# mit-gfx/recfilter

Hardware: AMD Instinct MI355X
Metric: Mpixels/s + achieved HBM GB/s, 16384^2 order-2 x/y Gaussian IIR (higher is better)
Workload: dtype f32; 1 GPU; cfg3: 16384x16384 f32 x1 plane(s) per GPU, 4 scans, clamped border; exchange=none, interior_beside_collective=False, steps_in_flight=1, backend=none, rccl_ranks=0

## Files before the change

include/recfilter_amd.h:

```cpp
#ifndef RECFILTER_AMD_H
#define RECFILTER_AMD_H

#include <stddef.h>
#include <stdint.h>

#ifdef __cplusplus
extern "C" {
#endif

#define RF_MAX_DIMS    3
#define RF_MAX_ORDER   32
#define RF_MAX_SCANS   32
#define RF_MAX_PLANES  16
#define RF_DEVICE_HOST_ONLY (-2)

typedef enum {
    RF_OK = 0,
    RF_ERR_INVALID_ARG = 1,
    RF_ERR_UNSUPPORTED = 2,
    RF_ERR_HIP = 3,
    RF_ERR_NOMEM = 4,
    RF_ERR_STATE = 5
} rf_status;

// ... 31 lines not shown
#define RF_PLAN_FORCE_EXCHANGE  0x01u
#define RF_PLAN_TILED_ONLY      0x02u
#define RF_PLAN_NO_CASCADE      0x04u
#define RF_PLAN_NO_SECTIONS     0x08u
#define RF_PLAN_NO_PLANE_BATCH  0x10u
#define RF_PLAN_STREAM_PASS1    0x20u
#define RF_PLAN_STAGED_PASS1    0x40u
#define RF_PLAN_LATE_EXCHANGE   0x80u
#define RF_PLAN_SERIAL_UNTILED  0x01000000u
#define RF_PLAN_MFMA_PASS1      0x02000000u
#define RF_PLAN_WALK_PASS1      0x04000000u
#define RF_PLAN_NO_OVERLAP      0x08000000u
#define RF_PLAN_INPLACE_Z       0x10000000u
#define RF_PLAN_FULL_CARRY_SCAN 0x20000000u
#define RF_PLAN_STAGE_HALF      0x40000000u
#define RF_PLAN_ALL_FLAGS       0x7f0000ffu
#define RF_PLAN_TILE_ROWS(n)    (((uint32_t)(n) & 0xffu) << 8)
#define RF_PLAN_TILE_PLANES(n)  (((uint32_t)(n) & 0xffu) << 16)

#define RF_ABI 3u

typedef struct {
    int32_t  ndim;
    uint32_t abi;
    int64_t  extent[RF_MAX_DIMS];
    int32_t  dtype;
    int32_t  n_planes;
    int32_t  border;
    int32_t  n_scans;
    const rf_scan_desc *scans;
    int32_t  tile[RF_MAX_DIMS];
// ... 71 lines not shown
```

recfilter_amd/capi.py:

```python
from __future__ import annotations

import ctypes
import os
import subprocess

_PKG = os.path.dirname(os.path.abspath(__file__))
LIB_PATH = os.environ.get("RECFILTER_AMD_LIB") or os.path.join(_PKG, "librecfilter_amd.so")
CSRC = os.path.join(_PKG, "csrc")

RF_MAX_DIMS = 3
RF_MAX_ORDER = 32
RF_ABI = 3
RF_MAX_SCANS = 32
RF_MAX_PLANES = 16
RF_DEVICE_HOST_ONLY = -2

RF_OK, RF_ERR_INVALID_ARG, RF_ERR_UNSUPPORTED, RF_ERR_HIP, RF_ERR_NOMEM, RF_ERR_STATE = range(6)
RF_F32, RF_F64, RF_I32, RF_I16, RF_F16, RF_BF16 = range(6)
RF_BORDER_ZERO, RF_BORDER_CLAMP = 0, 1
RF_POINTWISE_PRE, RF_POINTWISE_POST = 1, 2
RF_IN_PIXEL, RF_IN_U8, RF_IO_U8 = 0, 1, 2
RF_BUFFER_TABLE, RF_BUFFER_ZEROED, RF_BUFFER_SCRATCH = range(3)
BUFFER_KIND_NAMES = {RF_BUFFER_TABLE: "table", RF_BUFFER_ZEROED: "zeroed", RF_BUFFER_SCRATCH: "scratch"}
RF_PATH_AUTO, RF_PATH_UNTILED, RF_PATH_TILED_GENERIC, RF_PATH_TILED_FUSED, RF_PATH_TILED_OVERLAPPED, RF_PATH_TILED_MATRIX = range(6)
RF_PLAN_FORCE_EXCHANGE, RF_PLAN_TILED_ONLY, RF_PLAN_NO_CASCADE, RF_PLAN_NO_SECTIONS = 0x01, 0x02, 0x04, 0x08
RF_PLAN_NO_PLANE_BATCH, RF_PLAN_STREAM_PASS1, RF_PLAN_STAGED_PASS1, RF_PLAN_LATE_EXCHANGE = 0x10, 0x20, 0x40, 0x80
RF_PLAN_SERIAL_UNTILED = 0x01000000
RF_PLAN_MFMA_PASS1 = 0x02000000
RF_PLAN_WALK_PASS1 = 0x04000000
RF_PLAN_NO_OVERLAP = 0x08000000
RF_PLAN_INPLACE_Z = 0x10000000
RF_PLAN_FULL_CARRY_SCAN = 0x20000000
RF_PLAN_STAGE_HALF = 0x40000000


def RF_PLAN_TILE_ROWS(n: int) -> int:
    return (int(n) & 0xff) << 8


def RF_PLAN_TILE_PLANES(n: int) -> int:
    return (int(n) & 0xff) << 16


PATH_NAMES = {RF_PATH_AUTO: "auto", RF_PATH_UNTILED: "untiled",
              RF_PATH_TILED_GENERIC: "tiled_generic", RF_PATH_TILED_FUSED: "tiled_fused",
              RF_PATH_TILED_OVERLAPPED: "tiled_overlapped", RF_PATH_TILED_MATRIX: "tiled_matrix"}

EXPORTED_SYMBOLS = [
# ... 110 lines not shown
```

recfilter_amd/csrc/kernels_fused.h:

```cpp
#pragma once

#include <hip/hip_runtime.h>

#include <cstdint>

#include "kernels.h"
#include "pixel.h"
#include "rf_internal.h"

namespace rf {

constexpr int kFusedTX = 256;
constexpr int kFusedSeg = 16;
constexpr int kFusedThreads = 256;
constexpr int kFusedMaxK = 3;
constexpr int kFusedMaxMod = 8;
constexpr int kFusedMaxScans = 4;

template <typename Acc>
struct FusedScan {
    int32_t causal;
    Acc b;
    Acc a[kFusedMaxK];
    Acc R[kFusedMaxK][kFusedSeg];
// ... 36 lines not shown
    const Acc *y_nb_W;
    const Acc *x_incoming;
    int32_t pw_flags;
    Acc pre_s, pre_b, post_f, post_i, post_b;
    int32_t plane_batch;
    int32_t tx0, ty0, gx, gy;
    int32_t xcd_contig;
    int32_t mod_form;
    const void *in_planes[kFusedMaxPlanes];
    void *out_planes[kFusedMaxPlanes];
    int32_t yt_tile_major;
    int32_t yt_parts;
    int64_t yt_part_stride;
    const Acc *ytp;
    int64_t lin_limit;
    __host__ __device__ int64_t yt_index(int j, int ty, int r, int K, int64_t line) const {
        if (yt_tile_major)
            return ((((int64_t)ty * (NXP * NZ / kFusedTX) + (line >> 8)) * ny + j) * K + r) * kFusedTX + (line & 255);
        return (((int64_t)j * MY + ty) * K + r) * (NXP * NZ) + line;
    }
};

template <typename Acc>
struct StridedArgs {
    int64_t n, inner, lines;
    int32_t M;
    int32_t n_scans;
    int32_t clamped, first_is_border, last_is_border;
    int32_t mod_form;
    FusedScanY<Acc> scans[kFusedMaxScans];
// ... 47 lines not shown
int launch_fused_pass2_tall(int K, const void *src, int src_kind, P *dst, const FusedArgs<typename PixelTraits<P>::Acc> &a,
                            hipStream_t stream);
int launch_fused_pass2_u8(int K, int TY, const uint8_t *src, uint8_t *dst, const FusedArgs<float> &a, hipStream_t stream);
int launch_fused_pass2_tall_u8(int K, const uint8_t *src, uint8_t *dst, const FusedArgs<float> &a, hipStream_t stream);
template <typename P>
int launch_fused_tails(int K, int TY, const void *src, bool src_u8, const FusedArgs<typename PixelTraits<P>::Acc> &a,
                       const typename PixelTraits<P>::Acc *Hx, const typename PixelTraits<P>::Acc *Hy,
                       hipStream_t stream);
bool stream_tails_applicable(int K, int TY, bool src_u8, int pw_flags, int last_cols, int last_rows, int64_t n_tiles, int MX,
                             int64_t NZ, int nxk, int nyk, int mode );
int launch_stream_tails(int K, const float *src, const FusedArgs<float> &a, const float *Hx, const float *Hy, hipStream_t stream);
bool mfma_tails_applicable(int K, int TY, bool src_u8, int pw_flags, int last_cols, int last_rows, int64_t lin_limit, int nx, int ny,
                           int mode, bool narrow = false );
template <typename PI>
int launch_mfma_tails(int K, int TY, const PI *src, const FusedArgs<float> &a, const float *Hx, const float *Hy, hipStream_t stream);
struct WalkArgs {
    float *ytp;
    int64_t part_stride;
    float *zt;
    const float *HzT;
    int32_t TY, TZ, MZ;
    int32_t parts_log2;
    int32_t z_first_border, z_last_border;
    int32_t nzk, KZ;
    int32_t tall;
    float *xt2;
};
bool walk_tails_applicable(int K, int TY, int nx, int ny, int nz, int KZ, int TZ, int last_cols, int last_rows);
int launch_walk_tails(int K, const float *src, const FusedArgs<float> &a, const WalkArgs &wa, const float *Hx, const float *Hy,
                      hipStream_t stream);
// ... 6 lines not shown
```

recfilter_amd/csrc/kernels_fused_tall.hip:

```cpp
#include <atomic>
#include <type_traits>

#include "kernels.h"
#include "kernels_fused.h"
#include "scan_device.h"

namespace rf {

namespace {

constexpr int kTallTY = 128;
constexpr int kHalfRows = 64;

template <typename P, int K, bool EDGE, typename PI, int YPAT, bool EARLY, bool XFIX>
__global__ void __launch_bounds__(kFusedThreads, 2)
fused_pass2_tall_kernel(const PI *__restrict__ src, P *__restrict__ dst, FusedArgs<typename PixelTraits<P>::Acc> a) {
    using Acc = typename PixelTraits<P>::Acc;
    using A4 = typename Vec4<Acc>::type;
    extern __shared__ __attribute__((aligned(16))) unsigned char lds_raw[];
    Acc *tile = reinterpret_cast<Acc *>(lds_raw);
    A4 *tile4 = reinterpret_cast<A4 *>(lds_raw);
    constexpr int TY = kTallTY, TL = kHalfRows, NR = TL / 16;

    const int t = threadIdx.x;
    int bx = (int)blockIdx.x, by = (int)blockIdx.y;
    if (a.xcd_contig) {
        const unsigned gxn = gridDim.x, total = gxn * gridDim.y;
        unsigned b = (unsigned)by * gxn + (unsigned)bx;
        b = (b & 7u) * (total >> 3) + (b >> 3);
// ... 43 lines not shown
#pragma unroll
        for (int r = 0; r < K; r++) CY[j][r] = Acc(0);
        if (j < a.ny) {
            const bool causal = a.ys[j].causal != 0;
            const bool tile_first = causal ? (ty == 0) : (ty == a.MY - 1);
            if (tile_first) {
#pragma unroll
                for (int r = 0; r < K; r++) CY[j][r] = a.y_incoming[((int64_t)j * K + r) * Ly + line];
            } else {
                const int tp = causal ? ty - 1 : ty + 1;
#pragma unroll
                for (int r = 0; r < K; r++) CY[j][r] = a.yt[a.yt_index(j, tp, r, K, line)];
            }
        }
    }
    Acc yin[kFusedMaxScans][K];
    if (a.y_apply != nullptr) {
#pragma unroll
        for (int q = 0; q < kFusedMaxScans; q++)
#pragma unroll
            for (int o = 0; o < K; o++) yin[q][o] = q < a.ny ? a.y_incoming[((int64_t)q * K + o) * Ly + line] : Acc(0);
    } else if (a.y_nb_W != nullptr && ty < a.MY - 1) {
#pragma unroll
        for (int o = 0; o < K; o++) yin[0][o] = a.yt[a.yt_index(0, ty, o, K, line)];
    }
    auto apply_entering_carries = [&]() {
        if (a.y_nb_W != nullptr) {
            if (ty < a.MY - 1) {
                const int v = (ty + 1 == a.MY - 1) ? 2 : 0;
                const Acc *Wm = a.y_nb_W + ((v * a.ny + 0) * a.ny + 1) * K * K;
#pragma unroll
                for (int r = 0; r < K; r++)
#pragma unroll
                    for (int o = 0; o < K; o++) CY[1][r] = CY[1][r] + Wm[r * K + o] * yin[0][o];
            }
            return;
        }
        if (a.y_apply == nullptr) return;
#pragma unroll
        for (int j = 0; j < kFusedMaxScans; j++) {
            if (j < a.ny) {
// ... 7 lines not shown
#pragma unroll
                        for (int q = 0; q <= j; q++) {
                            const Acc *Ym = a.y_apply + ((((int64_t)q * a.ny + j) * a.MY + tp) * K + r) * K;
#pragma unroll
                            for (int o = 0; o < K; o++) add = add + Ym[o] * yin[q][o];
                        }
                        CY[j][r] = CY[j][r] + add;
                    }
                }
            }
        }
    };

    Acc *cx_lds = tile + TL * kFusedTX;
    Acc CX[2][kFusedMaxScans][NR][K];
#pragma unroll
    for (int h = 0; h < 2; h++) {
        const int64_t line0 = (int64_t)ty * TY + TL * h + slot + a.NYP * z;
#pragma unroll
        for (int s = 0; s < kFusedMaxScans; s++) {
#pragma unroll
            for (int n = 0; n < NR; n++)
#pragma unroll
                for (int j = 0; j < K; j++) CX[h][s][n][j] = Acc(0);
            if (s < a.nx) {
                const bool causal = a.xs[s].causal != 0;
                const bool tile_first = causal ? (tx == 0) : (tx == a.MX - 1);
                const bool first_lane = causal ? (l == 0) : (l == last_lane);
                if (first_lane) {
                    const int tp = causal ? tx - 1 : tx + 1;
                    const Acc *cp = tile_first ? a.x_incoming + (int64_t)s * K * Lx : a.xt + ((int64_t)s * a.MX + tp) * K * Lx;
#pragma unroll
                    for (int n = 0; n < NR; n++)
#pragma unroll
                        for (int j = 0; j < K; j++) CX[h][s][n][j] = cp[j * Lx + line0 + 16 * n];
                }
            }
        }
    }
    auto park_carries = [&]() {
#pragma unroll
        for (int h = 0; h < 2; h++)
#pragma unroll
            for (int s = 0; s < kFusedMaxScans; s++) {
                if (s < a.nx) {
                    const bool causal = a.xs[s].causal != 0;
                    const bool first_lane = causal ? (l == 0) : (l == last_lane);
                    if (first_lane) {
#pragma unroll
                        for (int n = 0; n < NR; n++)
#pragma unroll
                            for (int j = 0; j < K; j++) cx_lds[(((h * kFusedMaxScans + s) * NR + n) * K + j) * 16 + slot] = CX[h][s][n][j];
                    }
                }
            }
// ... 179 lines not shown
            } else
            if constexpr (packed_stores<P>::value) {
#pragma unroll
                for (int i = 0; i < TY; i += 2)
                    store_row_pair<P>(dpb, (uint32_t)t, (uint32_t)i, row_bytes, col[i], col[i + 1], (uint32_t)(EDGE ? rows_here : TY));
            } else
#pragma unroll
            for (int i = 0; i < TY; i++)
                if (!EDGE || i < rows_here)
                    __builtin_nontemporal_store(PixelTraits<P>::store(col[i]),
                                                reinterpret_cast<P *>(dpb + ((uint32_t)t * (uint32_t)sizeof(P) + (uint32_t)i * row_bytes)));
        }
    }
}

template <typename P, int K, bool EDGE, typename PI, int YPAT, bool EARLY, bool XFIX = false>
int launch_tall_pat(const PI *src, P *dst, const FusedArgs<typename PixelTraits<P>::Acc> &a, hipStream_t stream) {
    using Acc = typename PixelTraits<P>::Acc;
    const size_t lds = ((size_t)kHalfRows * kFusedTX + 2 * kFusedMaxScans * (kHalfRows / 16) * K * 16 + (size_t)a.ny * K * kFusedTX) * sizeof(Acc);
    const size_t lds_max = ((size_t)kHalfRows * kFusedTX + 2 * kFusedMaxScans * (kHalfRows / 16) * K * 16 + (size_t)kFusedMaxScans * K * kFusedTX) * sizeof(Acc);
    static std::atomic<bool> attr_set[64];
    int dev = 0;
    RF_HIP_CHECK(hipGetDevice(&dev));
    std::atomic<bool> &done = attr_set[dev & 63];
    if (!done.load(std::memory_order_acquire)) {
        RF_HIP_CHECK(hipFuncSetAttribute(reinterpret_cast<const void *>(&fused_pass2_tall_kernel<P, K, EDGE, PI, YPAT, EARLY, XFIX>),
                                         hipFuncAttributeMaxDynamicSharedMemorySize, (int)lds_max));
        done.store(true, std::memory_order_release);
    }
    dim3 grid((unsigned)(a.gx > 0 ? a.gx : a.MX), (unsigned)(a.gy > 0 ? a.gy : a.MY), (unsigned)a.NZ);
    FusedArgs<Acc> aa = a;
    aa.xcd_contig = (a.row_bytes % 128u != 0 && (grid.x * grid.y) % 8u == 0 && grid.x * grid.y >= 2048u) ? 1 : 0;
    hipLaunchKernelGGL((fused_pass2_tall_kernel<P, K, EDGE, PI, YPAT, EARLY, XFIX>), grid, dim3(kFusedThreads), lds, stream, src, dst, aa);
    RF_HIP_CHECK(hipGetLastError());
    return RF_OK;
}

template <typename P, int K, bool EDGE, typename PI>
int launch_tall_impl(const PI *src, P *dst, const FusedArgs<typename PixelTraits<P>::Acc> &a, hipStream_t stream) {
    const int pat = a.mod_form ? 0 : (a.ny == 1 && a.ys[0].causal != 0) ? 1 : (a.ny == 2 && a.ys[0].causal != 0 && a.ys[1].causal == 0) ? 2 : 0;
    bool early = !EDGE && pat > 0;
    if constexpr (!PixelTraits<P>::is_integer) early = early && (a.pw_flags & 2) == 0;
    const int xpat = a.mod_form ? 0 : (a.nx == 1 && a.xs[0].causal != 0) ? 1 : (a.nx == 2 && a.xs[0].causal != 0 && a.xs[1].causal == 0) ? 2 : 0;
    if constexpr (!EDGE) {
        if (early && pat == 1 && xpat == 1) return launch_tall_pat<P, K, EDGE, PI, 1, true, true>(src, dst, a, stream);
        if (early && pat == 2 && xpat == 2) return launch_tall_pat<P, K, EDGE, PI, 2, true, true>(src, dst, a, stream);
        if (early && pat == 1) return launch_tall_pat<P, K, EDGE, PI, 1, true>(src, dst, a, stream);
        if (early && pat == 2) return launch_tall_pat<P, K, EDGE, PI, 2, true>(src, dst, a, stream);
    }
    if (pat == 1) return launch_tall_pat<P, K, EDGE, PI, 1, false>(src, dst, a, stream);
    if (pat == 2) return launch_tall_pat<P, K, EDGE, PI, 2, false>(src, dst, a, stream);
    return launch_tall_pat<P, K, EDGE, PI, 0, false>(src, dst, a, stream);
}

template <int K, bool EDGE, typename PI>
int launch_tall_widen(const PI *src, float *dst, const FusedArgs<float> &a, hipStream_t stream) {
    if (a.mod_form || (a.pw_flags & 2) || a.plane_batch || a.y_nb_W != nullptr || a.y_apply != nullptr) {
        set_error("fused pass 2: a 16-bit source with an f32 destination is the x/y stage of an unsharded volume (no epilogue, no sections)");
// ... 100 lines not shown
```

recfilter_amd/csrc/kernels_tails.hip:

```cpp
#include <cstdlib>
#include <type_traits>

#include "kernels.h"
#include "kernels_fused.h"
#include "scan_device.h"

namespace rf {

namespace {


typedef float F2 __attribute__((ext_vector_type(2)));
typedef float F4 __attribute__((ext_vector_type(4)));

template <typename P, int K, int TY, typename PI, int MODE = 0, bool YM = false>
__global__ void __launch_bounds__(kFusedThreads)
fused_tails_kernel(const PI *__restrict__ src, FusedArgs<typename PixelTraits<P>::Acc> a,
                   const typename PixelTraits<P>::Acc *__restrict__ Hx,
                   const typename PixelTraits<P>::Acc *__restrict__ Hy) {
    using Acc = typename PixelTraits<P>::Acc;
    using A4 = typename Vec4<Acc>::type;
    constexpr int kTailRows = sizeof(Acc) == 8 ? 16 : 32;
    __shared__ __attribute__((aligned(16))) Acc tile[kTailRows * kFusedTX];
    extern __shared__ __attribute__((aligned(16))) unsigned char hx_raw[];
// ... 582 lines not shown
                const int64_t y = ybase + 4 * c4;
                A4 v = *reinterpret_cast<const A4 *>(a.xt + (((int64_t)s * a.MX + tx_i) * K + r) * Lx + y);
                if (s == 1 && tx_i > 0) {
                    const int vt = (tx_i == a.MX - 1) ? 2 : 0;
                    const Acc *Wm = Wx + ((vt * a.nx + 0) * a.nx + 1) * K * K + r * K;
#pragma unroll
                    for (int m = 0; m < K; m++) {
                        const A4 p = *reinterpret_cast<const A4 *>(a.xt + ((int64_t)(tx_i - 1) * K + m) * Lx + y);
                        const Acc w = Wm[m];
                        v.x = v.x + w * p.x; v.y = v.y + w * p.y; v.z = v.z + w * p.z; v.w = v.w + w * p.w;
                    }
                }
                *reinterpret_cast<A4 *>(xt_done + (((int64_t)s * a.MX + tx_i) * K + r) * Lx + y) = v;
            }
        }
    }
}

}

template <typename P>
int launch_fused_tails(int K, int TY, const void *src, bool src_u8, const FusedArgs<typename PixelTraits<P>::Acc> &a,
                       const typename PixelTraits<P>::Acc *Hx, const typename PixelTraits<P>::Acc *Hy,
                       hipStream_t stream) {
    if (a.MX <= 0 || a.MY <= 0 || a.NZ <= 0) return RF_OK;
    if (a.NZ > 65535 || a.MY > 65535) { set_error("fused path: grid too large"); return RF_ERR_UNSUPPORTED; }
    dim3 grid((unsigned)a.MX, (unsigned)a.MY, (unsigned)a.NZ);
    static const size_t pad_bytes = RF_KNOB("RF_TAILS_PAD_LDS") ? (size_t)atoi(RF_KNOB("RF_TAILS_PAD_LDS")) : 0;
    const size_t hx_bytes = (size_t)(a.nx > 0 ? a.nx : 1) * K * kFusedTX * sizeof(typename PixelTraits<P>::Acc) + pad_bytes;
    const size_t hy_bytes = (size_t)((a.ny * K + 3) & ~3) * 9 * 16;
// ... 125 lines not shown
            if (edge) RF_XSCAN_LAUNCH((Acc, KK, true, true), (Acc, KK, true, true, 0, true), dim3(grid), dim3(256), g_bytes, stream, a, gj, TY, Hy, G);  \
            else      RF_XSCAN_LAUNCH((Acc, KK, false, true), (Acc, KK, false, true, 0, true), dim3(grid), dim3(256), g_bytes, stream, a, gj, TY, Hy, G); \
        } else {                                                                                                           \
            if (edge) RF_XSCAN_LAUNCH((Acc, KK, true, false), (Acc, KK, true, false, 0, true), dim3(grid), dim3(256), g_bytes, stream, a, gj, TY, Hy, G);  \
            else      RF_XSCAN_LAUNCH((Acc, KK, false, false), (Acc, KK, false, false, 0, true), dim3(grid), dim3(256), g_bytes, stream, a, gj, TY, Hy, G); \
        }                                                                                                                  \
        RF_HIP_CHECK(hipGetLastError());                                                                                   \
        return RF_OK;                                                                                                      \
    }
    RF_CASE(1) RF_CASE(2) RF_CASE(3)
#undef RF_CASE
    set_error("xscan rows: unsupported order %d", K);
    return RF_ERR_UNSUPPORTED;
}

template int launch_fused_tails<float>(int, int, const void *, bool, const FusedArgs<float> &, const float *, const float *, hipStream_t);
template int launch_fused_tails<_Float16>(int, int, const void *, bool, const FusedArgs<float> &, const float *, const float *, hipStream_t);
template int launch_fused_tails<__bf16>(int, int, const void *, bool, const FusedArgs<float> &, const float *, const float *, hipStream_t);
template int launch_fused_tails<int32_t>(int, int, const void *, bool, const FusedArgs<uint32_t> &, const uint32_t *,
                                         const uint32_t *, hipStream_t);
template int launch_fused_tails<int16_t>(int, int, const void *, bool, const FusedArgs<uint32_t> &, const uint32_t *,
                                         const uint32_t *, hipStream_t);
template int launch_fused_tails<double>(int, int, const void *, bool, const FusedArgs<double> &, const double *, const double *, hipStream_t);
template int launch_xscan_rows<float>(int, int, const FusedArgs<float> &, const float *, const float *, hipStream_t, const float *, const float *, float *, bool);
template int launch_xscan_rows<uint32_t>(int, int, const FusedArgs<uint32_t> &, const uint32_t *, const uint32_t *, hipStream_t, const uint32_t *, const uint32_t *, uint32_t *, bool);
template int launch_xscan_rows<double>(int, int, const FusedArgs<double> &, const double *, const double *, hipStream_t, const double *, const double *, double *, bool);

}
```

recfilter_amd/csrc/kernels_tails_mfma.hip:

```cpp
#include <atomic>
#include <cstdlib>
#include <type_traits>

#include "kernels.h"
#include "kernels_fused.h"
#include "scan_device.h"

namespace rf {

namespace {

typedef float F2 __attribute__((ext_vector_type(2)));
typedef float F4 __attribute__((ext_vector_type(4)));

constexpr int kRows = 32;
constexpr int kHyPitch4 = 9;

__device__ __forceinline__ float sum_lanes_xor_16_32(float v) {
    typedef unsigned U2 __attribute__((ext_vector_type(2)));
    U2 r = __builtin_amdgcn_permlane16_swap(__float_as_uint(v), __float_as_uint(v), false, false);
    v = __uint_as_float(r[0]) + __uint_as_float(r[1]);
    r = __builtin_amdgcn_permlane32_swap(__float_as_uint(v), __float_as_uint(v), false, false);
    return __uint_as_float(r[0]) + __uint_as_float(r[1]);
}

__device__ __forceinline__ int row_swz(int row, int c) { return c ^ (row & 15) ^ ((c >> 4) & 3); }

template <int K, int TY, int NX, int NY, bool YM, typename PI = float>
__global__ void __launch_bounds__(kFusedThreads, 4)
mfma_tails_kernel(const PI *__restrict__ src, FusedArgs<float> a,
                  const float *__restrict__ Hx,
                  const float *__restrict__ Hy) {
    __shared__ __attribute__((aligned(16))) float tile[kRows * kFusedTX];
    extern __shared__ __attribute__((aligned(16))) unsigned char dyn_raw[];
    F4 *tile4 = reinterpret_cast<F4 *>(tile);
    float *stage = reinterpret_cast<float *>(dyn_raw);
    constexpr int NH = TY / kRows;
    constexpr int NL = kRows / 4;
    constexpr int NGX = NX > 0 ? (NX * K + 3) / 4 : 1;
    constexpr int NGY = NY > 0 ? (NY * K + 3) / 4 : 1;
    constexpr int NYK = NY > 0 ? NY * K : 1;

    const int t = threadIdx.x;
// ... 145 lines not shown
                                c0 = F2{h0[i], h0[i + 1]} * c2 + c0;
                                c1 = F2{h1[i], h1[i + 1]} * c2 + c1;
                            }
                            comb[2 * g] = comb[2 * g] + (c0.x + c0.y);
                            if (2 * g + 1 < NYK) comb[2 * g + 1] = comb[2 * g + 1] + (c1.x + c1.y);
                        }
                    }
                }
            }
        }
    }
    if (nxk > 0) {
        __syncthreads();
        flush_xtails(NH - 1);
    }
    if constexpr (YM) {
        if (nyk > 0) {
            const int64_t line = (int64_t)tx * kFusedTX + (t & ~3) + a.NXP * z;
#pragma unroll
            for (int g = 0; g < NGY; g++) {
                const int jr = 4 * g + (t & 3);
                if (jr < nyk) *reinterpret_cast<F4 *>(a.yt + a.yt_index(jr / K, ty, jr % K, K, line)) = yacc[g];
            }
        }
    } else if (nyk > 0) {
        const int64_t line = (int64_t)tx * kFusedTX + t + a.NXP * z;
#pragma unroll
        for (int jr = 0; jr < NYK; jr++)
            if (jr < nyk) a.yt[a.yt_index(jr / K, ty, jr % K, K, line)] = comb[jr];
    }
// ... 34 lines not shown
    if constexpr (std::is_same<PI, float>::value) {
        RF_CASES(1, 32) RF_CASES(1, 64) RF_CASES(1, 128)
        RF_CASES(2, 32) RF_CASES(2, 64) RF_CASES(2, 128)
        RF_CASES(3, 32) RF_CASES(3, 64) RF_CASES(3, 128)
    } else {
        RF_CASES_PAIRS(2, 32) RF_CASES_PAIRS(2, 64) RF_CASES_PAIRS(2, 128)
        RF_CASES_PAIRS(3, 32) RF_CASE(3, 64, 1, 1) RF_CASES_PAIRS(3, 128)
    }
#undef RF_CASES
#undef RF_CASES_PAIRS
#undef RF_CASE
    set_error("mfma tails: unsupported order %d / tile height %d / %d + %d scans", K, TY, a.nx, a.ny);
    return RF_ERR_UNSUPPORTED;
}

template int launch_mfma_tails<float>(int, int, const float *, const FusedArgs<float> &, const float *, const float *, hipStream_t);
template int launch_mfma_tails<_Float16>(int, int, const _Float16 *, const FusedArgs<float> &, const float *, const float *, hipStream_t);
template int launch_mfma_tails<__bf16>(int, int, const __bf16 *, const FusedArgs<float> &, const float *, const float *, hipStream_t);

}
```

recfilter_amd/csrc/plan_fused.cpp:

```cpp
#include <cmath>
#include <cstring>
#include <memory>

#include "kernels_fused.h"
#include "plan.h"
#include "plan_carry.h"
#include "plan_generic.h"
#include "plan_strided.h"

namespace rf {

namespace {

int fused_order(const rf_plan *plan) {
    return std::max(plan->dims[0].k, plan->ndim > 1 ? plan->dims[1].k : 0);
}

int64_t chained_padded_length(int64_t N) {
    if (N % 8192 == 0) return N;
    for (int64_t nx = 16384; nx >= kFusedTX; nx /= 2) {
        const int64_t g = nx * 32, np = (N + g - 1) / g * g;
        if (np - N <= N / 16) return np;
    }
    return (N + 8191) / 8192 * 8192;
// ... 121 lines not shown
    g.NX = NX; g.NY = NY; g.NZ = NZ; g.nx = nx; g.ny = ny;
    g.TY = TY; g.MX = MX; g.MY = MY; g.TVx = TVx; g.TVy = TVy;
    g.NXP = NXP; g.NYP = NYP; g.Lx = Lx; g.Ly = Ly;
    return g;
}

template <typename S, typename Acc>
struct FusedTables {
    CarryStage<S, Acc> x, y;
    std::vector<FusedScan<Acc>> xs, ys;
    const Acc *G = nullptr;
    const Acc *Hx = nullptr, *Hy = nullptr;
    const Acc *AMx = nullptr, *AMSx = nullptr;
    int chain_S = 1;
    bool nb_x = false, nb_y = false;
    bool nb_x_pair() const { return nb_x && x.n == 2; }
    bool nb_y_pair() const { return nb_y && y.n == 2; }
};

template <typename P, typename S>
int fused_tables(rf_plan *plan, const FusedGeometry &g, FusedTables<S, typename PixelTraits<P>::Acc> &t) {
    using Acc = typename PixelTraits<P>::Acc;
    using Options = typename CarryStage<S, Acc>::Options;
    int status = RF_OK;
    const int K = g.K, nx = g.nx, ny = g.ny;
    const DimInfo &dx = plan->dims[0];
    const DimInfo no_y;
    const DimInfo &dy = g.chained ? no_y : plan->dims[1];
    auto up = [&](const auto &vec) {
        using T = typename std::decay<decltype(vec)>::type::value_type;
// ... 49 lines not shown
                        dG[idx] = table_to_double<S>(Pm[(size_t)xi * K + o]);
                    }
            }
        plan->tables["G_x"] = dG;
    }
    if (ny > 0) {
        if (neighbour_plan) nb_bound_y = neighbour_carry_bound<S>(t.y.tab, dy.scan_ids, plan);
        hHy = table_for_kernels<S, Acc>(plan, build_tail_responses<S>(t.y.tab.scans, K, g.TY, plan->clamped, g.TVy), "H_y");
    }
    t.G = up(hG); t.Hx = up(hHx); t.Hy = up(hHy); t.AMx = up(hAMx); t.AMSx = up(hAMSx);

    const bool full_scan = (plan->flags & RF_PLAN_FULL_CARRY_SCAN) != 0;
    t.nb_x = !full_scan && nb_bound_x >= 0.0 && nb_bound_x <= kNeighbourCarryBound && (nx == 1 || ny > 0);
    t.nb_y = !full_scan && nb_bound_y >= 0.0 && nb_bound_y <= kNeighbourCarryBound && (ny == 1 || g.TY == 128);
    plan->tables["neighbour_carries"] = {nb_bound_x, t.nb_x ? 1.0 : 0.0, nb_bound_y, t.nb_y ? 1.0 : 0.0};
    return status;
}

template <typename Acc>
struct FusedBuffers {
    Acc *xt = nullptr, *yt = nullptr;
    Acc *xt_done = nullptr;
    Acc *xin = nullptr, *yin = nullptr;
    Acc *row_exit = nullptr;
    size_t xt_pp = 0, yt_pp = 0, xin_pp = 0, yin_pp = 0;
    bool merged_cx = false;
};

template <typename S, typename Acc>
int fused_buffers(rf_plan *plan, const FusedGeometry &g, FusedTables<S, Acc> &t, FusedBuffers<Acc> &b) {
// ... 83 lines not shown
        if (batch)
            for (int i = 0; i < plan->n_planes; i++) { a.in_planes[i] = plan->in[i]; a.out_planes[i] = plan->xy_result(i); }
        return a;
    }
};

template <typename Acc>
struct Pass1Args {
    int K = 0, TY = 0;
    const Acc *Hx = nullptr, *Hy = nullptr;
    bool padded = false;
    int stream_mode = 0, mfma_mode = 0;
    WalkArgs walk{};
    std::shared_ptr<WalkHook> walk_hook;
    size_t xt_pp = 0;
};

template <typename P>
int launch_pass1(const rf_plan *plan, int pl, const FusedArgs<typename PixelTraits<P>::Acc> &a,
                 const Pass1Args<typename PixelTraits<P>::Acc> &p) {
    const int K = p.K, TY = p.TY;
    const void *in = p.padded ? plan->pad_in[pl] : plan->in[pl];
    if constexpr (std::is_same<P, float>::value) {
        if (p.walk_hook) {
            WalkArgs wa = p.walk;
            wa.zt = p.walk_hook->zt + (size_t)pl * p.walk_hook->zt_stride;
            if (wa.xt2) wa.xt2 += (size_t)pl * p.xt_pp;
            if (wa.ytp) wa.ytp = const_cast<float *>(a.ytp);
            else wa.ytp = a.yt;
            return launch_walk_tails(K, (const float *)plan->in[pl], a, wa, p.Hx, p.Hy, plan->stream);
        }
        if (a.lin_limit == 0 && stream_tails_applicable(K, TY, plan->pw.in_u8, a.pw_flags, a.last_cols, a.last_rows, (int64_t)a.MX * a.MY * a.NZ, a.MX,
                                        a.NZ, a.nx * K, a.ny * K, p.stream_mode))
            return launch_stream_tails(K, (const float *)in, a, p.Hx, p.Hy, plan->stream);
        if (mfma_tails_applicable(K, TY, plan->pw.in_u8, a.pw_flags, a.last_cols, a.last_rows, a.lin_limit, a.nx, a.ny, p.mfma_mode))
            return launch_mfma_tails<float>(K, TY, (const float *)in, a, p.Hx, p.Hy, plan->stream);
    }
    if constexpr (is_half_pixel<P>::value) {
// ... 56 lines not shown
            for (int e = 0; e < kFusedMaxMod; e++) fbase.ys[j].mod_g[e] = t.ys[j].mod_g[e];
        }
        fargs.b = b;
        fargs.batch = g.batch;
        t.y.dev.base.tile_major = fbase.yt_tile_major;
    }

    int add_pass1() {
        int status = RF_OK;
        rf_plan *const plan = this->plan;
        Pass1Args<Acc> p1a;
        p1a.K = g.K; p1a.TY = g.TY; p1a.Hx = t.Hx; p1a.Hy = t.Hy; p1a.padded = g.padded;
        p1a.stream_mode = (plan->flags & RF_PLAN_STREAM_PASS1) ? 1 : (plan->flags & RF_PLAN_STAGED_PASS1) ? -1 : 0;
        p1a.mfma_mode = (plan->flags & RF_PLAN_MFMA_PASS1) ? 1 : (plan->flags & RF_PLAN_STAGED_PASS1) ? -1 : 0;
        p1a.walk = walk.args; p1a.walk_hook = walk.hook; p1a.xt_pp = b.xt_pp;
        Step p1;
        p1.name = walk.hook ? "walk_tails" : "fused_tails";
        p1.run = [plan, fargs = this->fargs, p1a](int pl) { return launch_pass1<P>(plan, pl, fargs(plan, pl), p1a); };
        if (g.padded) {
            plan->padded_len = g.N1;
            const size_t user_bytes = (size_t)plan->dims[0].N * sizeof(P);
            for (int pl = 0; pl < plan->n_planes; pl++) {
                plan->pad_in[pl] = plan->alloc((size_t)g.N1 * sizeof(P), true, &status);
                plan->pad_out[pl] = plan->alloc((size_t)g.N1 * sizeof(P), false, &status);
            }
            if (status != RF_OK) return status;
            Step ci;
            ci.name = "pad_copy_in";
            ci.run = [plan, user_bytes](int pl) -> int {
                RF_HIP_CHECK(hipMemcpyAsync(plan->pad_in[pl], plan->in[pl], user_bytes, hipMemcpyDeviceToDevice, plan->stream));
// ... 61 lines not shown
            ap.name = "carry_x_apply" + std::to_string(s);
            ap.run = [plan, cx, s](int pl) { return launch_generic_carry_apply<Acc>(cx.args(pl), s, plan->stream); };
            plan->begin_steps.push_back(ap);
        }
    }

    void add_xscan_rows() {
        rf_plan *const plan = this->plan;
        const int K = g.K, TY = g.TY;
        const bool merged_cx = b.merged_cx, nb_x_pair = t.nb_x_pair();
        const Acc *d_Hy = t.Hy, *d_G = t.G, *d_Wx = t.x.dev.base.W, *d_Ax = t.x.dev.base.A;
        Acc *const xt_done = b.xt_done;
        const size_t xt_pp = b.xt_pp;
        Step xs;
        xs.name = "xscan_rows";
        xs.run = [plan, fargs = this->fargs, K, TY, d_Hy, d_G, merged_cx, nb_x_pair, d_Wx, d_Ax, xt_done, xt_pp](int pl) {
            if (merged_cx)
                return launch_xscan_rows<Acc>(K, TY, fargs(plan, pl), d_Hy, d_G, plan->stream, d_Wx, d_Ax, xt_done + (size_t)pl * xt_pp);
            if (nb_x_pair)
                return launch_xscan_rows<Acc>(K, TY, fargs(plan, pl), d_Hy, d_G, plan->stream, d_Wx, nullptr, xt_done + (size_t)pl * xt_pp, true);
            return launch_xscan_rows<Acc>(K, TY, fargs(plan, pl), d_Hy, d_G, plan->stream);
        };
        plan->begin_steps.push_back(xs);
    }

    int add_y_carries() {
        if (!g.y_sharded) {
            if (g.ny > 0 && !t.nb_y) t.y.add_local_carry(plan, "carry_y");
            return RF_OK;
        }
        if (merged_exchange_applies(g.ny, g.K, plan->shard_world)) {
            static const bool separate_apply = RF_KNOB("RF_SHARD_SEPARATE_APPLY") != nullptr;
            return add_merged_exchange<S, Acc>(plan, t.y, "carry_y", separate_apply ? nullptr : &d_Yapply);
        }
        return t.y.add_per_scan_carries(plan, "carry_y", "carry_y_apply", true);
    }

    void add_pass2() {
        rf_plan *const plan = this->plan;
        const int K = g.K, TY = g.TY;
        const bool padded = g.padded;
        const Acc *d_Yapply = this->d_Yapply, *d_Ynb = t.nb_y_pair() ? t.y.dev.base.W : nullptr;
        Acc *const xt_done = (b.merged_cx || t.nb_x_pair()) ? b.xt_done : nullptr;
        const size_t xt_pp = b.xt_pp;
        Step p2;
        p2.name = "fused_pass2";
        p2.run = [plan, fargs = this->fargs, K, TY, d_Yapply, d_Ynb, padded, xt_done, xt_pp](int pl) {
            FusedArgs<Acc> a = fargs(plan, pl);
            a.y_apply = d_Yapply;
            a.y_nb_W = d_Ynb;
            if (xt_done) a.xt = xt_done + (size_t)pl * xt_pp;
            if constexpr (is_half_pixel<P>::value) {
                if (plan->mid[pl] != nullptr) {
                    const int kind = std::is_same<P, _Float16>::value ? kSrcF16 : kSrcBF16;
                    a.row_bytes = (uint32_t)(a.NX * (int64_t)sizeof(float));
                    if (TY == 128) return launch_fused_pass2_tall<float>(K, plan->in[pl], kind, (float *)plan->mid[pl], a, plan->stream);
                    return launch_fused_pass2<float>(K, TY, plan->in[pl], kind, (float *)plan->mid[pl], a, plan->stream);
                }
            }
            if constexpr (std::is_same<P, float>::value) {
                if (plan->pw.out_u8) {
                    a.row_bytes = (uint32_t)a.NX;
                    if (TY == 128) return launch_fused_pass2_tall_u8(K, (const uint8_t *)plan->in[pl], (uint8_t *)plan->out[pl], a, plan->stream);
                    return launch_fused_pass2_u8(K, TY, (const uint8_t *)plan->in[pl], (uint8_t *)plan->out[pl], a, plan->stream);
                }
            }
// ... 172 lines not shown
```

Measured before the change: 483,600 Mpixels/s.

## Fold x-carry effects into y tails via per-tile tau row-scan form

Adds a default-on 'row scans' form for order-2 causal/anticausal x and y pairs with neighbour carries. Pass 1 scans the combined y-tail rows in x inside the MFMA tails kernel. A new xtau kernel then reduces the x carries against Hy into small per-tile 4Kx4K tau blocks, replacing the full xscan_rows pass. Pass 2 rebuilds the y entering carries from tau and a G table, and applies the x neighbour correction locally. The goal is to cut the traffic and latency of the intermediate x-carry pass, at the cost of more per-thread register arithmetic and state in pass 2.

```diff
diff --git a/include/recfilter_amd.h b/include/recfilter_amd.h
--- a/include/recfilter_amd.h
+++ b/include/recfilter_amd.h
@@ -69,7 +69,8 @@
 #define RF_PLAN_INPLACE_Z       0x10000000u
 #define RF_PLAN_FULL_CARRY_SCAN 0x20000000u
 #define RF_PLAN_STAGE_HALF      0x40000000u
-#define RF_PLAN_ALL_FLAGS       0x7f0000ffu
+#define RF_PLAN_SEPARATE_ROW_SCANS 0x80000000u
+#define RF_PLAN_ALL_FLAGS       0xff0000ffu
 #define RF_PLAN_TILE_ROWS(n)    (((uint32_t)(n) & 0xffu) << 8)
 #define RF_PLAN_TILE_PLANES(n)  (((uint32_t)(n) & 0xffu) << 16)
 
diff --git a/recfilter_amd/capi.py b/recfilter_amd/capi.py
--- a/recfilter_amd/capi.py
+++ b/recfilter_amd/capi.py
@@ -32,6 +32,7 @@
 RF_PLAN_INPLACE_Z = 0x10000000
 RF_PLAN_FULL_CARRY_SCAN = 0x20000000
 RF_PLAN_STAGE_HALF = 0x40000000
+RF_PLAN_SEPARATE_ROW_SCANS = 0x80000000
 
 
 def RF_PLAN_TILE_ROWS(n: int) -> int:
diff --git a/recfilter_amd/csrc/kernels_fused.h b/recfilter_amd/csrc/kernels_fused.h
--- a/recfilter_amd/csrc/kernels_fused.h
+++ b/recfilter_amd/csrc/kernels_fused.h
@@ -74,6 +74,9 @@
     int64_t yt_part_stride;
     const Acc *ytp;
     int64_t lin_limit;
+    const Acc *x_nb_W;
+    const Acc *rs_tau;
+    const Acc *rs_G;
     __host__ __device__ int64_t yt_index(int j, int ty, int r, int K, int64_t line) const {
         if (yt_tile_major)
             return ((((int64_t)ty * (NXP * NZ / kFusedTX) + (line >> 8)) * ny + j) * K + r) * kFusedTX + (line & 255);
@@ -151,6 +154,8 @@
                            int mode, bool narrow = false );
 template <typename PI>
 int launch_mfma_tails(int K, int TY, const PI *src, const FusedArgs<float> &a, const float *Hx, const float *Hy, hipStream_t stream);
+int launch_mfma_tails_row_scans(const float *src, const FusedArgs<float> &a, const float *Hx, const float *Hy, hipStream_t stream);
+int launch_xtau(const FusedArgs<float> &a, const float *Hy, const float *Wx, float *tau, hipStream_t stream);
 struct WalkArgs {
     float *ytp;
     int64_t part_stride;
diff --git a/recfilter_amd/csrc/kernels_fused_tall.hip b/recfilter_amd/csrc/kernels_fused_tall.hip
--- a/recfilter_amd/csrc/kernels_fused_tall.hip
+++ b/recfilter_amd/csrc/kernels_fused_tall.hip
@@ -12,7 +12,7 @@
 constexpr int kTallTY = 128;
 constexpr int kHalfRows = 64;
 
-template <typename P, int K, bool EDGE, typename PI, int YPAT, bool EARLY, bool XFIX>
+template <typename P, int K, bool EDGE, typename PI, int YPAT, bool EARLY, bool XFIX, bool RS = false>
 __global__ void __launch_bounds__(kFusedThreads, 2)
 fused_pass2_tall_kernel(const PI *__restrict__ src, P *__restrict__ dst, FusedArgs<typename PixelTraits<P>::Acc> a) {
     using Acc = typename PixelTraits<P>::Acc;
@@ -86,6 +86,24 @@
             }
         }
     }
+    Acc rs_g[RS ? 2 * K : 1];
+    Acc rs_t[RS ? 3 : 1][K][RS ? 2 * K : 1];
+    if constexpr (RS) {
+        static_assert(!EDGE && YPAT == 2 && XFIX && std::is_same<Acc, float>::value, "row scans: whole tiles, the pair in x and in y");
+        const int vx = (tx == 0 ? 1 : 0) | (tx == a.MX - 1 ? 2 : 0);
+#pragma unroll
+        for (int qo = 0; qo < 2 * K; qo++) rs_g[qo] = a.rs_G[((size_t)vx * 2 * K + qo) * kFusedTX + t];
+        const int64_t tile_id = (z * a.MY + ty) * a.MX + tx;
+        const Acc *tp = a.rs_tau + tile_id * (4 * K * K);
+#pragma unroll
+        for (int r = 0; r < K; r++)
+#pragma unroll
+            for (int qo = 0; qo < 2 * K; qo++) {
+                rs_t[0][r][qo] = ty > 0 ? tp[-(int64_t)a.MX * (4 * K * K) + r * 2 * K + qo] : Acc(0);
+                rs_t[1][r][qo] = ty < a.MY - 1 ? tp[r * 2 * K + qo] : Acc(0);
+                rs_t[2][r][qo] = ty < a.MY - 1 ? tp[(int64_t)a.MX * (4 * K * K) + (K + r) * 2 * K + qo] : Acc(0);
+            }
+    }
     Acc yin[kFusedMaxScans][K];
     if (a.y_apply != nullptr) {
 #pragma unroll
@@ -97,6 +115,18 @@
         for (int o = 0; o < K; o++) yin[0][o] = a.yt[a.yt_index(0, ty, o, K, line)];
     }
     auto apply_entering_carries = [&]() {
+        if constexpr (RS) {
+#pragma unroll
+            for (int r = 0; r < K; r++)
+#pragma unroll
+                for (int qo = 0; qo < 2 * K; qo++) {
+                    if (ty > 0) CY[0][r] = CY[0][r] + rs_g[qo] * rs_t[0][r][qo];
+                    if (ty < a.MY - 1) {
+                        yin[0][r] = yin[0][r] + rs_g[qo] * rs_t[1][r][qo];
+                        CY[1][r] = CY[1][r] + rs_g[qo] * rs_t[2][r][qo];
+                    }
+                }
+        }
         if (a.y_nb_W != nullptr) {
             if (ty < a.MY - 1) {
                 const int v = (ty + 1 == a.MY - 1) ? 2 : 0;
@@ -134,6 +164,7 @@
 
     Acc *cx_lds = tile + TL * kFusedTX;
     Acc CX[2][kFusedMaxScans][NR][K];
+    Acc XOWN[RS ? 2 : 1][RS ? NR : 1][K];
 #pragma unroll
     for (int h = 0; h < 2; h++) {
         const int64_t line0 = (int64_t)ty * TY + TL * h + slot + a.NYP * z;
@@ -154,11 +185,34 @@
                     for (int n = 0; n < NR; n++)
 #pragma unroll
                         for (int j = 0; j < K; j++) CX[h][s][n][j] = cp[j * Lx + line0 + 16 * n];
+                    if constexpr (RS) {
+                        if (s == 1 && !tile_first) {
+                            const Acc *op = a.xt + (int64_t)tx * K * Lx;
+#pragma unroll
+                            for (int n = 0; n < NR; n++)
+#pragma unroll
+                                for (int j = 0; j < K; j++) XOWN[h][n][j] = op[j * Lx + line0 + 16 * n];
+                        }
+                    }
                 }
             }
         }
     }
     auto park_carries = [&]() {
+        if constexpr (RS) {
+            if (l == last_lane && tx < a.MX - 1) {
+                const int vt = (tx + 1 == a.MX - 1) ? 2 : 0;
+                const Acc *Wm = a.x_nb_W + ((vt * 2 + 0) * 2 + 1) * K * K;
+#pragma unroll
+                for (int h = 0; h < 2; h++)
+#pragma unroll
+                    for (int n = 0; n < NR; n++)
+#pragma unroll
+                        for (int j = 0; j < K; j++)
+#pragma unroll
+                            for (int m = 0; m < K; m++) CX[h][1][n][j] = CX[h][1][n][j] + Wm[j * K + m] * XOWN[h][n][m];
+            }
+        }
 #pragma unroll
         for (int h = 0; h < 2; h++)
 #pragma unroll
@@ -368,7 +422,7 @@
     }
 }
 
-template <typename P, int K, bool EDGE, typename PI, int YPAT, bool EARLY, bool XFIX = false>
+template <typename P, int K, bool EDGE, typename PI, int YPAT, bool EARLY, bool XFIX = false, bool RS = false>
 int launch_tall_pat(const PI *src, P *dst, const FusedArgs<typename PixelTraits<P>::Acc> &a, hipStream_t stream) {
     using Acc = typename PixelTraits<P>::Acc;
     const size_t lds = ((size_t)kHalfRows * kFusedTX + 2 * kFusedMaxScans * (kHalfRows / 16) * K * 16 + (size_t)a.ny * K * kFusedTX) * sizeof(Acc);
@@ -378,14 +432,14 @@
     RF_HIP_CHECK(hipGetDevice(&dev));
     std::atomic<bool> &done = attr_set[dev & 63];
     if (!done.load(std::memory_order_acquire)) {
-        RF_HIP_CHECK(hipFuncSetAttribute(reinterpret_cast<const void *>(&fused_pass2_tall_kernel<P, K, EDGE, PI, YPAT, EARLY, XFIX>),
+        RF_HIP_CHECK(hipFuncSetAttribute(reinterpret_cast<const void *>(&fused_pass2_tall_kernel<P, K, EDGE, PI, YPAT, EARLY, XFIX, RS>),
                                          hipFuncAttributeMaxDynamicSharedMemorySize, (int)lds_max));
         done.store(true, std::memory_order_release);
     }
     dim3 grid((unsigned)(a.gx > 0 ? a.gx : a.MX), (unsigned)(a.gy > 0 ? a.gy : a.MY), (unsigned)a.NZ);
     FusedArgs<Acc> aa = a;
     aa.xcd_contig = (a.row_bytes % 128u != 0 && (grid.x * grid.y) % 8u == 0 && grid.x * grid.y >= 2048u) ? 1 : 0;
-    hipLaunchKernelGGL((fused_pass2_tall_kernel<P, K, EDGE, PI, YPAT, EARLY, XFIX>), grid, dim3(kFusedThreads), lds, stream, src, dst, aa);
+    hipLaunchKernelGGL((fused_pass2_tall_kernel<P, K, EDGE, PI, YPAT, EARLY, XFIX, RS>), grid, dim3(kFusedThreads), lds, stream, src, dst, aa);
     RF_HIP_CHECK(hipGetLastError());
     return RF_OK;
 }
@@ -396,6 +450,14 @@
     bool early = !EDGE && pat > 0;
     if constexpr (!PixelTraits<P>::is_integer) early = early && (a.pw_flags & 2) == 0;
     const int xpat = a.mod_form ? 0 : (a.nx == 1 && a.xs[0].causal != 0) ? 1 : (a.nx == 2 && a.xs[0].causal != 0 && a.xs[1].causal == 0) ? 2 : 0;
+    if (a.rs_tau != nullptr) {
+        if constexpr (!EDGE && K == 2 && std::is_same<P, float>::value && std::is_same<PI, float>::value) {
+            if (early && pat == 2 && xpat == 2 && a.y_nb_W != nullptr && a.x_nb_W != nullptr && a.rs_G != nullptr && a.y_apply == nullptr)
+                return launch_tall_pat<P, K, EDGE, PI, 2, true, true, true>(src, dst, a, stream);
+        }
+        set_error("fused pass 2: the row-scan form is misconfigured");
+        return RF_ERR_INVALID_ARG;
+    }
     if constexpr (!EDGE) {
         if (early && pat == 1 && xpat == 1) return launch_tall_pat<P, K, EDGE, PI, 1, true, true>(src, dst, a, stream);
         if (early && pat == 2 && xpat == 2) return launch_tall_pat<P, K, EDGE, PI, 2, true, true>(src, dst, a, stream);
diff --git a/recfilter_amd/csrc/kernels_tails.hip b/recfilter_amd/csrc/kernels_tails.hip
--- a/recfilter_amd/csrc/kernels_tails.hip
+++ b/recfilter_amd/csrc/kernels_tails.hip
@@ -620,6 +620,84 @@
                 *reinterpret_cast<A4 *>(xt_done + (((int64_t)s * a.MX + tx_i) * K + r) * Lx + y) = v;
             }
         }
+    }
+}
+
+template <int K>
+__global__ void __launch_bounds__(256)
+xtau_kernel(FusedArgs<float> a, const float *__restrict__ Hy, const float *__restrict__ Wx, float *__restrict__ tau) {
+    typedef float A4 __attribute__((ext_vector_type(4)));
+    constexpr int TY = 128, NXK = 2 * K, NYK = 2 * K;
+    const int t = threadIdx.x;
+    const int l = t & 15, row = t >> 4;
+    const int n_xg = (a.MX + 15) / 16;
+    int b = blockIdx.x;
+    const int xg = b % n_xg; b /= n_xg;
+    const int64_t z = b % a.NZ;
+    const int ty = (int)(b / a.NZ);
+    const int tx = xg * 16 + row;
+    const bool row_ok = tx < a.MX;
+    float tv[NYK][NXK];
+#pragma unroll
+    for (int jr = 0; jr < NYK; jr++)
+#pragma unroll
+        for (int qo = 0; qo < NXK; qo++) tv[jr][qo] = 0.0f;
+    if (row_ok) {
+        const int vy = ((ty == 0 && a.y_first_border) ? 1 : 0) | ((ty == a.MY - 1 && a.y_last_border) ? 2 : 0);
+        const int64_t Lx = a.NYP * a.NZ;
+        const A4 zero4 = A4{0.0f, 0.0f, 0.0f, 0.0f};
+#pragma unroll
+        for (int blk = 0; blk < TY; blk += 64) {
+            A4 hy[NYK];
+#pragma unroll
+            for (int jr = 0; jr < NYK; jr++) hy[jr] = *reinterpret_cast<const A4 *>(Hy + (size_t)(vy * NYK + jr) * TY + blk + 4 * l);
+            const int64_t y0 = (int64_t)ty * TY + a.NYP * z + blk + 4 * l;
+            A4 own[K];
+#pragma unroll
+            for (int o = 0; o < K; o++)
+                own[o] = tx < a.MX - 1 ? *reinterpret_cast<const A4 *>(a.xt + ((int64_t)tx * K + o) * Lx + y0) : zero4;
+#pragma unroll
+            for (int q = 0; q < 2; q++) {
+                const bool qc = q == 0;
+                const bool q_first = qc ? (tx == 0) : (tx == a.MX - 1);
+                const int tp = qc ? tx - 1 : tx + 1;
+#pragma unroll
+                for (int o = 0; o < K; o++) {
+                    A4 c = zero4;
+                    if (!q_first) c = *reinterpret_cast<const A4 *>(a.xt + (((int64_t)q * a.MX + tp) * K + o) * Lx + y0);
+                    if (q == 1 && !q_first) {
+                        const int vn = (tx + 1 == a.MX - 1) ? 2 : 0;
+                        const float *Wm = Wx + ((vn * 2 + 0) * 2 + 1) * K * K + o * K;
+#pragma unroll
+                        for (int m = 0; m < K; m++) {
+                            const float w = Wm[m];
+                            c.x = c.x + w * own[m].x; c.y = c.y + w * own[m].y;
+                            c.z = c.z + w * own[m].z; c.w = c.w + w * own[m].w;
+                        }
+                    }
+#pragma unroll
+                    for (int jr = 0; jr < NYK; jr++)
+                        tv[jr][q * K + o] = tv[jr][q * K + o] + (hy[jr].x * c.x + hy[jr].y * c.y + hy[jr].z * c.z + hy[jr].w * c.w);
+                }
+            }
+        }
+    }
+#pragma unroll
+    for (int jr = 0; jr < NYK; jr++)
+#pragma unroll
+        for (int qo = 0; qo < NXK; qo++) {
+            tv[jr][qo] = tv[jr][qo] + dpp_move<0xB1>(tv[jr][qo]);
+            tv[jr][qo] = tv[jr][qo] + dpp_move<0x4E>(tv[jr][qo]);
+            tv[jr][qo] = tv[jr][qo] + dpp_move<0x141>(tv[jr][qo]);
+            tv[jr][qo] = tv[jr][qo] + dpp_move<0x140>(tv[jr][qo]);
+        }
+    if (row_ok && l == 0) {
+        float *dst = tau + ((z * a.MY + ty) * a.MX + tx) * (NYK * NXK);
+#pragma unroll
+        for (int jr = 0; jr < NYK; jr++)
+#pragma unroll
+            for (int qo = 0; qo < NXK; qo += 4)
+                *reinterpret_cast<A4 *>(dst + jr * NXK + qo) = A4{tv[jr][qo], tv[jr][qo + 1], tv[jr][qo + 2], tv[jr][qo + 3]};
     }
 }
 
@@ -775,6 +853,20 @@
     return RF_ERR_UNSUPPORTED;
 }
 
+int launch_xtau(const FusedArgs<float> &a, const float *Hy, const float *Wx, float *tau, hipStream_t stream) {
+    if (a.MY <= 0 || a.MX <= 0 || a.NZ <= 0) return RF_OK;
+    if (Hy == nullptr || Wx == nullptr || tau == nullptr || a.nx != 2 || a.ny != 2 || a.mod_form || a.xs[0].causal == 0 || a.xs[1].causal != 0 ||
+        a.last_rows != 128 || a.last_cols != kFusedTX) {
+        set_error("xtau: the row-scan form is misconfigured");
+        return RF_ERR_INVALID_ARG;
+    }
+    const int64_t blocks = (int64_t)a.MY * a.NZ * ((a.MX + 15) / 16);
+    if (blocks >= (1ll << 31)) { set_error("xtau: grid too large"); return RF_ERR_UNSUPPORTED; }
+    hipLaunchKernelGGL((xtau_kernel<2>), dim3((unsigned)blocks), dim3(256), 0, stream, a, Hy, Wx, tau);
+    RF_HIP_CHECK(hipGetLastError());
+    return RF_OK;
+}
+
 template int launch_fused_tails<float>(int, int, const void *, bool, const FusedArgs<float> &, const float *, const float *, hipStream_t);
 template int launch_fused_tails<_Float16>(int, int, const void *, bool, const FusedArgs<float> &, const float *, const float *, hipStream_t);
 template int launch_fused_tails<__bf16>(int, int, const void *, bool, const FusedArgs<float> &, const float *, const float *, hipStream_t);
diff --git a/recfilter_amd/csrc/kernels_tails_mfma.hip b/recfilter_amd/csrc/kernels_tails_mfma.hip
--- a/recfilter_amd/csrc/kernels_tails_mfma.hip
+++ b/recfilter_amd/csrc/kernels_tails_mfma.hip
@@ -26,7 +26,7 @@
 
 __device__ __forceinline__ int row_swz(int row, int c) { return c ^ (row & 15) ^ ((c >> 4) & 3); }
 
-template <int K, int TY, int NX, int NY, bool YM, typename PI = float>
+template <int K, int TY, int NX, int NY, bool YM, typename PI = float, bool RS = false>
 __global__ void __launch_bounds__(kFusedThreads, 4)
 mfma_tails_kernel(const PI *__restrict__ src, FusedArgs<float> a,
                   const float *__restrict__ Hx,
@@ -202,6 +202,41 @@
         __syncthreads();
         flush_xtails(NH - 1);
     }
+    if constexpr (RS) {
+        static_assert(!YM && NX > 0 && NY > 0 && std::is_same<PI, float>::value, "row scans: f32 planes, both dimensions filtered");
+        const int e = (swz_chunk(t >> 2) << 2) | (t & 3);
+#pragma unroll
+        for (int jr = 0; jr < NYK; jr++) tile[jr * kFusedTX + e] = comb[jr];
+        __syncthreads();
+        static_assert(NYK <= 4, "row scans: one wave holds the combined rows");
+        if (w == 0 && (lane >> 4) < NYK) {
+            const int l = lane & 15, row = lane >> 4, sw = (l >> 2) & 3;
+            float v[1][kFusedSeg];
+#pragma unroll
+            for (int j = 0; j < 4; j++) {
+                const F4 q = tile4[row * 64 + 4 * l + (j ^ sw)];
+                v[0][4 * j + 0] = q.x; v[0][4 * j + 1] = q.y; v[0][4 * j + 2] = q.z; v[0][4 * j + 3] = q.w;
+            }
+            float zero[1][K];
+#pragma unroll
+            for (int j = 0; j < K; j++) zero[0][j] = 0.0f;
+#pragma unroll 1
+            for (int s = 0; s < NX; s++) {
+                const FusedScan<float> &sc = a.xs[s];
+                const bool causal = sc.causal != 0;
+                const bool tile_first = causal ? (tx == 0) : (tx == a.MX - 1);
+                const bool first_lane = causal ? (l == 0) : (l == 15);
+                const bool clamp_first = a.clamped && tile_first && first_lane;
+                if (causal) scan_rows16<float, true, K, 1>(v, sc, first_lane, clamp_first, zero);
+                else        scan_rows16<float, false, K, 1>(v, sc, first_lane, clamp_first, zero, false, kFusedSeg);
+            }
+            float *dst = a.yt + a.yt_index(row / K, ty, row % K, K, (int64_t)tx * kFusedTX + a.NXP * z) + 16 * l;
+#pragma unroll
+            for (int j = 0; j < 4; j++)
+                *reinterpret_cast<F4 *>(dst + 4 * j) = F4{v[0][4 * j + 0], v[0][4 * j + 1], v[0][4 * j + 2], v[0][4 * j + 3]};
+        }
+        return;
+    }
     if constexpr (YM) {
         if (nyk > 0) {
             const int64_t line = (int64_t)tx * kFusedTX + (t & ~3) + a.NXP * z;
@@ -266,6 +301,21 @@
     return RF_ERR_UNSUPPORTED;
 }
 
+int launch_mfma_tails_row_scans(const float *src, const FusedArgs<float> &a, const float *Hx, const float *Hy, hipStream_t stream) {
+    if (a.MX <= 0 || a.MY <= 0 || a.NZ <= 0) return RF_OK;
+    if (a.NZ > 65535 || a.MY > 65535) { set_error("fused path: grid too large"); return RF_ERR_UNSUPPORTED; }
+    if (a.nx != 2 || a.ny != 2 || a.last_cols != kFusedTX || a.last_rows != 128 || a.lin_limit != 0 || a.mod_form || (a.pw_flags & 1) ||
+        a.xs[0].causal == 0 || a.xs[1].causal != 0 || a.yt_parts > 1) {
+        set_error("mfma tails: the row-scan form is misconfigured");
+        return RF_ERR_INVALID_ARG;
+    }
+    dim3 grid((unsigned)a.MX, (unsigned)a.MY, (unsigned)a.NZ);
+    const size_t stage_bytes = (size_t)4 * 4 * kRows * sizeof(float);
+    hipLaunchKernelGGL((mfma_tails_kernel<2, 128, 2, 2, false, float, true>), grid, dim3(kFusedThreads), stage_bytes, stream, src, a, Hx, Hy);
+    RF_HIP_CHECK(hipGetLastError());
+    return RF_OK;
+}
+
 template int launch_mfma_tails<float>(int, int, const float *, const FusedArgs<float> &, const float *, const float *, hipStream_t);
 template int launch_mfma_tails<_Float16>(int, int, const _Float16 *, const FusedArgs<float> &, const float *, const float *, hipStream_t);
 template int launch_mfma_tails<__bf16>(int, int, const __bf16 *, const FusedArgs<float> &, const float *, const float *, hipStream_t);
diff --git a/recfilter_amd/csrc/plan_fused.cpp b/recfilter_amd/csrc/plan_fused.cpp
--- a/recfilter_amd/csrc/plan_fused.cpp
+++ b/recfilter_amd/csrc/plan_fused.cpp
@@ -159,6 +159,7 @@
     const Acc *AMx = nullptr, *AMSx = nullptr;
     int chain_S = 1;
     bool nb_x = false, nb_y = false;
+    bool row_scans = false;
     bool nb_x_pair() const { return nb_x && x.n == 2; }
     bool nb_y_pair() const { return nb_y && y.n == 2; }
 };
@@ -238,6 +239,17 @@
     t.nb_x = !full_scan && nb_bound_x >= 0.0 && nb_bound_x <= kNeighbourCarryBound && (nx == 1 || ny > 0);
     t.nb_y = !full_scan && nb_bound_y >= 0.0 && nb_bound_y <= kNeighbourCarryBound && (ny == 1 || g.TY == 128);
     plan->tables["neighbour_carries"] = {nb_bound_x, t.nb_x ? 1.0 : 0.0, nb_bound_y, t.nb_y ? 1.0 : 0.0};
+
+    if constexpr (std::is_same<P, float>::value) {
+        const int mfma_mode = (plan->flags & RF_PLAN_MFMA_PASS1) ? 1 : (plan->flags & RF_PLAN_STAGED_PASS1) ? -1 : 0;
+        const int stream_mode = (plan->flags & RF_PLAN_STREAM_PASS1) ? 1 : (plan->flags & RF_PLAN_STAGED_PASS1) ? -1 : 0;
+        t.row_scans = !(plan->flags & RF_PLAN_SEPARATE_ROW_SCANS) && t.nb_x_pair() && t.nb_y_pair() && K == 2 && g.TY == 128 &&
+                      g.TVx == kFusedTX && g.TVy == 128 && !plan->pw.in_u8 && !plan->pw.out_u8 && !plan->pw.pre && !plan->pw.post &&
+                      !g.padded && !g.in_place_tail && t.xs[0].causal != 0 && t.xs[1].causal == 0 && t.ys[0].causal != 0 && t.ys[1].causal == 0 &&
+                      !stream_tails_applicable(K, g.TY, false, 0, g.TVx, g.TVy, (int64_t)g.MX * g.MY * g.NZ, g.MX, g.NZ, nx * K, ny * K, stream_mode) &&
+                      mfma_tails_applicable(K, g.TY, false, 0, g.TVx, g.TVy, 0, nx, ny, mfma_mode);
+    }
+    plan->tables["row_scans"] = {t.row_scans ? 1.0 : 0.0};
     return status;
 }
 
@@ -351,6 +363,7 @@
     WalkArgs walk{};
     std::shared_ptr<WalkHook> walk_hook;
     size_t xt_pp = 0;
+    bool row_scans = false;
 };
 
 template <typename P>
@@ -359,6 +372,7 @@
     const int K = p.K, TY = p.TY;
     const void *in = p.padded ? plan->pad_in[pl] : plan->in[pl];
     if constexpr (std::is_same<P, float>::value) {
+        if (p.row_scans) return launch_mfma_tails_row_scans((const float *)in, a, p.Hx, p.Hy, plan->stream);
         if (p.walk_hook) {
             WalkArgs wa = p.walk;
             wa.zt = p.walk_hook->zt + (size_t)pl * p.walk_hook->zt_stride;
@@ -445,6 +459,7 @@
         p1a.stream_mode = (plan->flags & RF_PLAN_STREAM_PASS1) ? 1 : (plan->flags & RF_PLAN_STAGED_PASS1) ? -1 : 0;
         p1a.mfma_mode = (plan->flags & RF_PLAN_MFMA_PASS1) ? 1 : (plan->flags & RF_PLAN_STAGED_PASS1) ? -1 : 0;
         p1a.walk = walk.args; p1a.walk_hook = walk.hook; p1a.xt_pp = b.xt_pp;
+        p1a.row_scans = t.row_scans;
         Step p1;
         p1.name = walk.hook ? "walk_tails" : "fused_tails";
         p1.run = [plan, fargs = this->fargs, p1a](int pl) { return launch_pass1<P>(plan, pl, fargs(plan, pl), p1a); };
@@ -536,6 +551,15 @@
         const size_t xt_pp = b.xt_pp;
         Step xs;
         xs.name = "xscan_rows";
+        if constexpr (std::is_same<Acc, float>::value) {
+            if (t.row_scans) {
+                xs.run = [plan, fargs = this->fargs, d_Hy, d_Wx, xt_done, xt_pp](int pl) {
+                    return launch_xtau(fargs(plan, pl), d_Hy, d_Wx, xt_done + (size_t)pl * xt_pp, plan->stream);
+                };
+                plan->begin_steps.push_back(xs);
+                return;
+            }
+        }
         xs.run = [plan, fargs = this->fargs, K, TY, d_Hy, d_G, merged_cx, nb_x_pair, d_Wx, d_Ax, xt_done, xt_pp](int pl) {
             if (merged_cx)
                 return launch_xscan_rows<Acc>(K, TY, fargs(plan, pl), d_Hy, d_G, plan->stream, d_Wx, d_Ax, xt_done + (size_t)pl * xt_pp);
@@ -565,13 +589,16 @@
         const Acc *d_Yapply = this->d_Yapply, *d_Ynb = t.nb_y_pair() ? t.y.dev.base.W : nullptr;
         Acc *const xt_done = (b.merged_cx || t.nb_x_pair()) ? b.xt_done : nullptr;
         const size_t xt_pp = b.xt_pp;
+        const bool row_scans = t.row_scans;
+        const Acc *d_Xnb = row_scans ? t.x.dev.base.W : nullptr, *d_G = row_scans ? t.G : nullptr;
         Step p2;
         p2.name = "fused_pass2";
-        p2.run = [plan, fargs = this->fargs, K, TY, d_Yapply, d_Ynb, padded, xt_done, xt_pp](int pl) {
+        p2.run = [plan, fargs = this->fargs, K, TY, d_Yapply, d_Ynb, padded, xt_done, xt_pp, row_scans, d_Xnb, d_G](int pl) {
             FusedArgs<Acc> a = fargs(plan, pl);
             a.y_apply = d_Yapply;
             a.y_nb_W = d_Ynb;
-            if (xt_done) a.xt = xt_done + (size_t)pl * xt_pp;
+            if (row_scans) { a.x_nb_W = d_Xnb; a.rs_G = d_G; a.rs_tau = xt_done + (size_t)pl * xt_pp; }
+            else if (xt_done) a.xt = xt_done + (size_t)pl * xt_pp;
             if constexpr (is_half_pixel<P>::value) {
                 if (plan->mid[pl] != nullptr) {
                     const int kind = std::is_same<P, _Float16>::value ? kSrcF16 : kSrcBF16;
```

Measured after the change: 500,300 Mpixels/s, median of 6. 3.5% higher.
